# madmann91/bvh

Hardware: AMD Instinct MI355X
Metric: Mrays/s closest-hit (1M-tri scene) (higher is better)
Workload: dtype f32; 1 GPU; soup_1m: 1,000,000-triangle random soup (M3), worst-case incoherent; robust traversal, DefaultBuilder with thread pool (mini-trees) Quality::High built on the GPU (the reference's default configuration is thread pool + High); rays reordered for coherence inside the timed pass (library default for this tree size); tris=1000000, nodes=1866439, ray_batches=4, parallelism=single GPU, launched_by=single process

## Files before the change

bvh_amd/__init__.py:

```python
from .api import (BinnedSahBuilder, MiniTreeBuilder, SplitHeuristic, Bvh, Config, DefaultBuilder, Quality, RayFlags, SweepSahBuilder, ThreadPool, prepare_trace,
                  HITD, HITF, INVALID, NODED, NODEF, NODE2D, NODE2F, closest_points, hits_to_numpy, intersect, precompute_tris, sphere_bounds,
                  tri_bounds, gather, radius_count, radius_search, offsets_from_counts, knn, KNN_MAX_K, std_sort_ids, radix_sort_pairs, reinsertion_stats, last_optimize_profile, pinhole_rays, shade_eyelight)
from ._lib import BvhAmdError
```

bvh_amd/_lib.py:

```python
from __future__ import annotations

import ctypes as C
import os

HERE = os.path.dirname(os.path.abspath(__file__))
LIB_PATH = os.environ.get("BVH_AMD_LIB") or os.path.join(HERE, "lib", "libbvh_amd.so")

_lib = None


class BvhAmdError(RuntimeError):
    pass


class BuildConfig(C.Structure):
    _fields_ = [("quality", C.c_int), ("min_leaf_size", C.c_size_t), ("max_leaf_size", C.c_size_t),
                ("parallel_threshold", C.c_size_t)]


class Counters(C.Structure):
    _fields_ = [("node_pairs", C.c_ulonglong), ("prim_tests", C.c_ulonglong), ("leaves", C.c_ulonglong)]


class MiniTreeConfig(C.Structure):
# ... 106 lines not shown
    "bvh{S}_get_prim_id": (_Z, [_P, _Z]),
    "bvh{S}_get_prim_count": (_Z, [_P]),
    "bvh{S}_get_node_count": (_Z, [_P]),
    "bvh_node{S}_is_leaf": (C.c_bool, [_P]),
    "bvh_node{S}_get_prim_count": (_Z, [_P]),
    "bvh_node{S}_get_first_id": (_Z, [_P]),
    "bvh{S}_copy_nodes": (None, [_P, _P]),
    "bvh{S}_copy_prim_ids": (None, [_P, _P]),
    "bvh{S}_device_prim_ids": (_P, [_P]),
    "bvh_amd_tri_bounds{S}": (_I, [_P, _Z, _P, _P, _P]),
    "bvh_amd_precompute_tris{S}": (_I, [_P, _P, _Z, _P, _P]),
    "bvh_amd_sphere_bounds{S}": (_I, [_P, _Z, _P, _P, _P]),
    "bvh{S}_intersect_rays_tri": (_I, [_P, _P, _P, _Z, _U, _P, _P, _P]),
    "bvh{S}_intersect_rays_sphere": (_I, [_P, _P, _P, _Z, _U, _P, _P, _P]),
    "bvh{S}_prepare_trace": (_I, [_P, _Z, _P]),
    "bvh{S}_closest_points_tri": (_I, [_P, _P, _P, _Z, _U, _P, _P, _P]),
    "bvh{S}_closest_points_sphere": (_I, [_P, _P, _P, _Z, _U, _P, _P, _P]),
    "bvh{S}_radius_search_tri": (_I, [_P, _P, _P, _Z, _U, _P, _P, _P, _P, _P, _P]),
    "bvh{S}_radius_search_sphere": (_I, [_P, _P, _P, _Z, _U, _P, _P, _P, _P, _P, _P]),
    "bvh{S}_knn_tri": (_I, [_P, _P, _P, _Z, _U, _U, _P, _P, _P, _P, _P]),
    "bvh{S}_knn_sphere": (_I, [_P, _P, _P, _Z, _U, _U, _P, _P, _P, _P, _P]),
    "bvh{S}_intersect_ray": (None, [_P, _P, _P]),
    "bvh{S}_intersect_ray_any": (None, [_P, _P, _P]),
    "bvh{S}_intersect_ray_robust": (None, [_P, _P, _P]),
    "bvh{S}_intersect_ray_any_robust": (None, [_P, _P, _P]),
    "bvh{S}_intersect_ray_visit": (_I, [_P, _P, _Z, _U, _P]),
}


class OptimizeProfile(C.Structure):
# ... 6 lines not shown

class OptimizeConfig(C.Structure):
    _fields_ = [("batch_size_ratio", C.c_double), ("max_iter_count", C.c_size_t)]


def ray_visitor_types(suffix: str):
    scalar = C.c_float if suffix[1] == "f" else C.c_double
    leaf_t = C.CFUNCTYPE(C.c_bool, C.c_void_p, C.POINTER(scalar), C.c_size_t, C.c_size_t)
    inner_t = C.CFUNCTYPE(None, C.c_void_p, C.c_size_t)

    class Visitor(C.Structure):
        _fields_ = [("user_data", C.c_void_p), ("leaf_fn", leaf_t), ("inner_fn", inner_t)]
    return Visitor, leaf_t, inner_t


_ONLY_3D = ("bvh_amd_tri_bounds{S}", "bvh_amd_precompute_tris{S}", "bvh{S}_intersect_rays_tri", "bvh{S}_prepare_trace",
            "bvh{S}_build_minitree_device",
            "bvh{S}_closest_points_tri", "bvh{S}_closest_points_sphere",
            "bvh{S}_radius_search_tri", "bvh{S}_radius_search_sphere",
            "bvh{S}_knn_tri", "bvh{S}_knn_sphere",
            "bvh{S}_refit_tris", "bvh{S}_traversal_cost")


def exported_symbols():
    names = list(_SIGS)
    for s in ("3f", "3d", "2f", "2d"):
        names += [k.format(S=s) for k in _SIGS_T if s[0] == "3" or k not in _ONLY_3D]
        names += [f"bvh_node{s}_get_bbox"]
    return names


# ... 34 lines not shown
```

bvh_amd/api.py:

```python
from __future__ import annotations

import ctypes as C
import enum
from dataclasses import dataclass, field

import numpy as np

from . import _lib

INVALID = 0xFFFFFFFF
HITF = np.dtype([("prim", "<u4"), ("t", "<f4"), ("u", "<f4"), ("v", "<f4")])
HITD = np.dtype([("prim", "<u4"), ("pad", "<u4"), ("t", "<f8"), ("u", "<f8"), ("v", "<f8")])
NODEF = np.dtype([("bounds", "<f4", (6,)), ("index", "<u4")])
NODED = np.dtype([("bounds", "<f8", (6,)), ("index", "<u8")])
NODE2F = np.dtype([("bounds", "<f4", (4,)), ("index", "<u4")])
NODE2D = np.dtype([("bounds", "<f8", (4,)), ("index", "<u8")])
_NODE_DTYPES = {"3f": NODEF, "3d": NODED, "2f": NODE2F, "2d": NODE2D}


class Quality(enum.IntEnum):
    Low = 0
    Medium = 1
    High = 2

# ... 396 lines not shown

def gather(records, perm):
    torch = _torch()
    r = _dev(records)
    p = _dev(perm).to(torch.int32)
    out = torch.empty((p.shape[0],) + tuple(r.shape[1:]), dtype=r.dtype, device=r.device)
    stride = r.element_size() * int(np.prod(r.shape[1:]))
    _lib.check(_lib.load().bvh_amd_gather(r.data_ptr(), p.data_ptr(), p.shape[0], stride, out.data_ptr(), _stream()), "gather")
    return out


def prepare_trace(bvh: Bvh, n_rays_hint: int = 0):
    if bvh.dim != 3:
        return
    _lib.check(getattr(_lib.load(), f"bvh{bvh._s}_prepare_trace")(bvh._h, int(n_rays_hint), _stream()), "prepare_trace")


def intersect(bvh: Bvh, prims, rays, any_hit: bool = False, robust: bool = False, leaf: str = "tri",
              counters: bool = False, out=None, sort_rays=None, original_ids: bool = False):
    torch = _torch()
    lib = _lib.load()
    s = bvh._s
    dt = torch.float32 if s[1] == "f" else torch.float64
    r = _dev(rays, 2 * bvh.dim + 2)
    p = _dev(prims)
    if bvh.dim == 2:
        leaf = "sphere"
    if r.dtype != dt or p.dtype != dt:
        raise TypeError("prims/rays dtype must match the BVH scalar type")
    n = r.shape[0]
# ... 209 lines not shown
```

bvh_amd/csrc/capi.hip:

```cpp
#include "common.h"

#include <cstring>
#include <memory>

namespace bvh_amd {

template <typename T> int reinsertion_optimize_device(HostNode<T>* d_nodes, size_t node_count, hipStream_t stream, int dim);
template <typename T>
int reinsertion_optimize_config_device(HostNode<T>* d_nodes, size_t node_count, hipStream_t stream, int dim, double batch_size_ratio, size_t iterations);
void reinsertion_stats(unsigned out[2]);
void last_optimize_profile(bvh_amd_optimize_profile* out);
template <typename T>
int build_minitree_explicit(BvhImpl<T>& out, const T* d_bboxes, const T* d_centers, size_t n, const bvh_build_config& cfg, bool prune, T ratio,
                            bool optimize, uint32_t log2_grid, hipStream_t stream);
template <typename T>
int extract_device(BvhImpl<T>& out, const HostNode<T>* d_nodes, size_t node_count, const uint32_t* d_ids, size_t root_id, hipStream_t stream);
template <typename T> int refit_device(HostNode<T>* d_nodes, size_t node_count, hipStream_t stream);
template <typename T> int reachable_node_count(const HostNode<T>* d_nodes, size_t node_count, hipStream_t stream, size_t* out);
template <typename T> int relayout_on_device(BvhImpl<T>& b, const HostNode<T>* d_nodes, hipStream_t stream);

namespace {
thread_local std::string g_error;
}

// ... 289 lines not shown
        return fail(BVH_AMD_ERR_ARG, std::string(who) + ": " + std::to_string(n_src) + " primitives given, but prim_ids refers to primitive " +
                    std::to_string(b.max_prim_id) + " (the array is indexed by original primitive id)");
    const bool from_host = b.host_valid || !b.d_nodes || b.d_nodes_count != b.node_count;
    int rc = from_host ? b.wait_refit() : BVH_AMD_OK;
    if (rc) return rc;
    rc = make_nodes_resident<T>(b);
    if (rc) return rc;
    if (from_host || (b.pair_count && !b.d_pairs)) {
        const long long largest = b.max_prim_id;
        rc = relayout_on_device<T>(b, b.d_nodes, stream);
        if (rc) return rc;
        b.max_prim_id = largest;
    }
    rc = refit_prims_device<T>(b.d_nodes, b.d_pairs, b.node_count, src_kind, d_src, n_src, b.d_prim_ids, b.prim_count, stream);
    if (rc == BVH_AMD_OK && d_tris12_out) rc = launch_precompute_tris<T>(d_src, b.d_prim_ids, b.prim_count, d_tris12_out, stream);
    b.host_valid = false;
    b.nodes2_valid = false;
    const int rc2 = b.note_refit(stream);
    return rc ? rc : rc2;
}

template <typename T>
int traversal_cost_checked(const BvhImpl<T>* b, double* cost_out, void* stream) {
    if (!b || !cost_out) return fail(BVH_AMD_ERR_ARG, "traversal_cost: null bvh or output");
    int cur = -1;
    BVH_HIP_TRY(hipGetDevice(&cur), BVH_AMD_ERR_HIP);
    if (cur != b->device) return fail(BVH_AMD_ERR_ARG, "traversal_cost: BVH lives on another device than the current one");
    return traversal_cost<T>(*b, cost_out, static_cast<hipStream_t>(stream));
}

// ... 407 lines not shown
        return radius_search<T>(b, LEAF_TRIANGLE, prims, queries, n, flags, counts, offsets, list_prims, list_dist, cnt, s); } \
    int bvh##S##_radius_search_sphere(const bvh##S* b, const T* prims, const T* queries, size_t n, unsigned flags, uint32_t* counts, \
                                      const uint64_t* offsets, uint32_t* list_prims, T* list_dist, bvh_amd_counters* cnt, void* s) { \
        return radius_search<T>(b, LEAF_SPHERE, prims, queries, n, flags, counts, offsets, list_prims, list_dist, cnt, s); } \
    int bvh##S##_knn_tri(const bvh##S* b, const T* prims, const T* queries, size_t n, unsigned k, unsigned flags, uint32_t* out_prims, \
                         T* out_dist, uint32_t* counts, bvh_amd_counters* cnt, void* s) {                           \
        return knn<T>(b, LEAF_TRIANGLE, prims, queries, n, k, flags, out_prims, out_dist, counts, cnt, s); }        \
    int bvh##S##_knn_sphere(const bvh##S* b, const T* prims, const T* queries, size_t n, unsigned k, unsigned flags, uint32_t* out_prims, \
                            T* out_dist, uint32_t* counts, bvh_amd_counters* cnt, void* s) {                        \
        return knn<T>(b, LEAF_SPHERE, prims, queries, n, k, flags, out_prims, out_dist, counts, cnt, s); }          \
    int bvh##S##_prepare_trace(const bvh##S* b, size_t n_rays_hint, void* s) {                                      \
        if (!b) return fail(BVH_AMD_ERR_ARG, "prepare_trace: null bvh");                                            \
        int cur = -1;                                                                                               \
        BVH_HIP_TRY(hipGetDevice(&cur), BVH_AMD_ERR_HIP);                                                           \
        if (cur != impl<T>(b)->device) return fail(BVH_AMD_ERR_ARG, "prepare_trace: BVH lives on another device than the current one"); \
        return prepare_trace<T>(*impl<T>(b), n_rays_hint, static_cast<hipStream_t>(s)); }

BVH_AMD_IMPL(float, 3f)
BVH_AMD_IMPL(double, 3d)

#define BVH_AMD_IMPL_RAY(T, S, CB, VIS, D, IMPL)                                                                         \
    void bvh##S##_intersect_ray(const bvh##S* b, const bvh_ray##S* r, const CB* cb) { intersect_ray_legacy<T, D>(IMPL<T>(b), r, cb, 0u); } \
    void bvh##S##_intersect_ray_any(const bvh##S* b, const bvh_ray##S* r, const CB* cb) {                           \
        intersect_ray_legacy<T, D>(IMPL<T>(b), r, cb, BVH_AMD_RAY_ANY_HIT); }                                        \
    void bvh##S##_intersect_ray_robust(const bvh##S* b, const bvh_ray##S* r, const CB* cb) {                        \
        intersect_ray_legacy<T, D>(IMPL<T>(b), r, cb, BVH_AMD_RAY_ROBUST); }                                         \
    void bvh##S##_intersect_ray_any_robust(const bvh##S* b, const bvh_ray##S* r, const CB* cb) {                    \
        intersect_ray_legacy<T, D>(IMPL<T>(b), r, cb, BVH_AMD_RAY_ANY_HIT | BVH_AMD_RAY_ROBUST); }                   \
    int bvh##S##_intersect_ray_visit(const bvh##S* b, const bvh_ray##S* r, size_t start, unsigned flags, const VIS* v) { \
        if (!v || !v->leaf_fn) return fail(BVH_AMD_ERR_ARG, "intersect_ray_visit: null visitor");                   \
        return intersect_ray_visit<T, D>(IMPL<T>(b), r, start, flags, v->leaf_fn, v->inner_fn, v->user_data); }
// ... 127 lines not shown
```

bvh_amd/csrc/common.h:

```cpp
#pragma once

#include <hip/hip_runtime.h>

#include <cstddef>
#include <cstdint>
#include <cstring>
#include <string>
#include <atomic>
#include <mutex>
#include <vector>

#include "../../include/bvh_amd.h"

namespace bvh_amd {

constexpr unsigned kCountBits = 4;
constexpr uint32_t kCountMask = 15u;
constexpr int kWave = 64;

template <typename T> struct IndexOf;
template <> struct IndexOf<float>  { using Type = uint32_t; };
template <> struct IndexOf<double> { using Type = uint64_t; };

template <typename T>
// ... 69 lines not shown
    int sync_host() const;
    HostNode<T>* h_root = nullptr;
    hipEvent_t refit_done = nullptr;
    mutable std::atomic<bool> root_pending{false};
    mutable std::mutex root_mutex;
    int wait_refit() const;
    int note_refit(hipStream_t stream);
    long long max_prim_id = -1;
    int device = -1;
    PairNode<T>* d_pairs = nullptr;
    size_t pair_count = 0;
    uint32_t* d_prim_ids = nullptr;
    uint32_t root_index = 0;
    mutable std::atomic<int> max_depth{-1};
    mutable std::atomic<float> expected_visits{0.0f};
    mutable std::atomic<uint32_t> launch_plan[2] = {};
    struct PlanSearch {
        int index = 0;
        static constexpr int kCandidates = 5;
        int trying = -1;
        uint8_t count[kCandidates] = {};
        uint8_t dropped = 0;
        bool pending = false;
        bool recorded = false;
        hipEvent_t start = nullptr, stop = nullptr;
        size_t rays = 0;
        float ns_per_ray[kCandidates] = {};
        size_t rays_of[kCandidates] = {};
    };
    mutable PlanSearch plan_search[2];
// ... 132 lines not shown
```

bvh_amd/csrc/trace_body.inc:

```
#ifndef BVH_TRACE_COOP
#define BVH_TRACE_COOP false
#endif
    constexpr int kDepth = kLdsDepth;
    constexpr int kSpill = 64 - kDepth;
    __shared__ uint32_t lds_stack[kDepth * kBlock];
    uint32_t spill[kSpill];
    const int tid = threadIdx.x;
    const int lane = tid & (kWave - 1);
    const uint64_t lanes_below = (uint64_t{1} << lane) - 1;

    bool have = false, done = false, drained = false, nan_ray = false;
    uint32_t part = a.parts > 1 ? blockIdx.x % a.parts : 0, parts_left = a.parts;
    unsigned long long ray_id = 0;
    T org[3], dir[3], inv[3], aux[3];
    T tmin = 0, tmax = 0;
    uint32_t oct[3] = {0, 0, 0};
    uint32_t top = 0, sp = 0;
    uint32_t hit_prim = BVH_AMD_INVALID;
    T hit_t = 0, hit_u = 0, hit_v = 0;
    unsigned long long n_pairs = 0, n_tests = 0, n_leaves = 0;
#if defined(BVH_AMD_DEVELOPER) && defined(__HIPCC__)
    unsigned long long wt_begin = 0, wt_last_refill = 0, wt_rays = 0, wt_refill_ticks = 0, wt_refills = 0;
    if (a.wave_times) wt_begin = __builtin_amdgcn_s_memrealtime();
#endif

    auto deep_slot = [&](uint32_t i) { return a.deep + (size_t{blockIdx.x} * kBlock + tid) * a.deep_cap + i; };
    auto push = [&](uint32_t v) {
        if (sp < kDepth) lds_stack[sp * kBlock + tid] = v;
        else if (!Deep) spill[min(sp - kDepth, static_cast<uint32_t>(kSpill - 1))] = v;
        else if (sp < kDepth + kSpill) spill[sp - kDepth] = v;
        else *deep_slot(min(sp - (kDepth + kSpill), a.deep_cap - 1)) = v;
        ++sp;
    };
    auto pop = [&]() -> uint32_t {
        --sp;
        uint32_t v = lds_word(&lds_stack[min(sp, static_cast<uint32_t>(kDepth - 1)) * kBlock + tid]);
        if (sp >= kDepth) {
            if (!Deep) v = spill[min(sp - kDepth, static_cast<uint32_t>(kSpill - 1))];
            else if (sp < kDepth + kSpill) v = spill[sp - kDepth];
            else v = *deep_slot(min(sp - (kDepth + kSpill), a.deep_cap - 1));
        }
        return v;
    };

    for (;;) {
        const uint64_t idle = __ballot(!have);
        const int n_idle = __popcll(idle);
        if (!drained && (n_idle >= a.refill_threshold || n_idle == kWave)) {
#if defined(BVH_AMD_DEVELOPER) && defined(__HIPCC__)
            unsigned long long wt_t0 = 0;
            if (a.wave_times) wt_t0 = __builtin_amdgcn_s_memrealtime();
// ... 51 lines not shown
                wt_refill_ticks += wt_last_refill - wt_t0; ++wt_refills;
            }
#endif
        }
        if (__ballot(have) == 0) {
            if (drained) break;
            continue;
        }

        for (;;) {
            const bool inner = have && !done && (top & kCountMask) == 0;
            const uint64_t inner_mask = __ballot(inner);
            if (!inner_mask) break;
            const int parked = __popcll(__ballot(have && !done && (top & kCountMask) != 0));
            if (parked >= a.leaf_threshold) break;
            T lb[6], rb[6];
            uint32_t li = 0, ri = 0;
            if constexpr (BVH_TRACE_COOP) coop_load_pair(a.pairs, a.pair_bytes, inner ? (top >> (kCountBits + 1)) : 0xFFFFFFFFu, lane, lb, rb, li, ri);
            if (inner) {
                if constexpr (!BVH_TRACE_COOP) load_pair(a.pairs + (top >> (kCountBits + 1)), lb, rb, li, ri);
                if (Stats) ++n_pairs;
                T l0 = tmin, l1 = tmax, r0 = tmin, r1 = tmax;
#pragma unroll
                for (int k = 0; k < D; ++k) {
                    const T ln = oct[k] ? lb[2 * k + 1] : lb[2 * k], lf = oct[k] ? lb[2 * k] : lb[2 * k + 1];
                    const T rn = oct[k] ? rb[2 * k + 1] : rb[2 * k], rf = oct[k] ? rb[2 * k] : rb[2 * k + 1];
                    T la, lz, ra, rz;
                    if (Robust) {
                        la = (ln - org[k]) * inv[k]; lz = (lf - org[k]) * aux[k];
                        ra = (rn - org[k]) * inv[k]; rz = (rf - org[k]) * aux[k];
                    } else {
                        la = Num<T>::fma_(ln, inv[k], aux[k]); lz = Num<T>::fma_(lf, inv[k], aux[k]);
                        ra = Num<T>::fma_(rn, inv[k], aux[k]); rz = Num<T>::fma_(rf, inv[k], aux[k]);
                    }
                    l0 = Num<T>::max_num(la, l0); l1 = Num<T>::min_num(lz, l1);
                    r0 = Num<T>::max_num(ra, r0); r1 = Num<T>::min_num(rz, r1);
                }
                const bool hl = !nan_ray && l0 <= l1, hr = !nan_ray && r0 <= r1;
                if (hl) {
                    uint32_t near_i = li;
                    if (hr) {
                        uint32_t far_i = ri;
                        if (!Any && l0 > r0) { near_i = ri; far_i = li; }
                        push(far_i);
                    }
                    top = near_i;
                } else if (hr) {
                    top = ri;
                } else if (sp == 0) {
                    done = true;
                } else {
                    top = pop();
                }
            }
        }

        if (have && !done && (top & kCountMask) != 0) {
            const uint32_t first = top >> kCountBits, count = top & kCountMask;
            if (Stats) ++n_leaves;
// ... 77 lines not shown
```

bvh_amd/csrc/trace_device.h:

```cpp
#pragma once

#if defined(__HIPCC__)
#define BVH_AMD_KEEP_APART(v) asm volatile("" : "+v"(v))
#else
#define BVH_AMD_KEEP_APART(v) asm volatile("" : "+r"(v))
#endif

namespace bvh_amd {

namespace {

constexpr int kBlock = 256;
constexpr int kLdsDepth = 20;
constexpr int kRefillThreshold = 36;
constexpr int kRefillThresholdSmall = 20;
constexpr int kLeafThreshold = 12;
constexpr int kCoopRefillAny = 20, kCoopLeafAny = 20;
constexpr int kCoopRefillHeavy = 12, kCoopLeafHeavy = 12;


template <typename T> struct Num;
template <> struct Num<float> {
    static constexpr float kMax = 3.402823466e+38f, kEps = 1.1920928955078125e-07f;
    __device__ static bool finite(float x) { return (__float_as_uint(x) & 0x7F800000u) != 0x7F800000u; }
    __device__ static float bump2(float x) { return __uint_as_float(__float_as_uint(x) + 2u); }
    __device__ static bool sign(float x) { return (__float_as_uint(x) >> 31) != 0; }
    __device__ static float fma_(float a, float b, float c) { return __builtin_fmaf(a, b, c); }
    __device__ static float sqrt_(float x) { return __builtin_sqrtf(x); }
// ... 20 lines not shown
template <typename T> __device__ inline T pick_min(T a, T b) { return a < b ? a : b; }
template <typename T> __device__ inline T pick_max(T a, T b) { return a > b ? a : b; }

template <typename T> __device__ inline T dot3(T a0, T a1, T a2, T b0, T b1, T b2) {
    return ((T(0) + a0 * b0) + a1 * b1) + a2 * b2;
}
__device__ inline uint32_t lds_word(const uint32_t* shared) {
#if defined(__HIP_DEVICE_COMPILE__)
    typedef __attribute__((address_space(3))) const volatile uint32_t LdsWord;
    return *(LdsWord*)shared;
#else
    return *shared;
#endif
}

template <typename T> __device__ inline T dot2(T a0, T a1, T b0, T b1) { return (T(0) + a0 * b0) + a1 * b1; }

constexpr uint32_t kTicketStride = 16;

template <typename T>
struct TraceArgs {
    const PairNode<T>* pairs;
    const T* prims;
    const T* rays;
    typename HitOf<T>::Type* hits;
    unsigned long long n;
    unsigned long long* work;
    unsigned long long part_size;
    uint32_t parts;
    bvh_amd_counters* counters;
    const uint32_t* order;
    uint32_t* deep;
    uint32_t deep_cap;
    uint32_t root_index;
    int refill_threshold;
    int leaf_threshold;
    uint32_t coop;
    uint32_t prim_stride;
    uint32_t stream_hints;
    uint32_t stagger;
    uint32_t one_shot;
    unsigned long long* wave_times;
    uint32_t pair_bytes = 0;
};

__device__ inline void load_pair(const PairNode<float>* p, float (&lb)[6], float (&rb)[6], uint32_t& li, uint32_t& ri) {
    const float4* q = reinterpret_cast<const float4*>(p);
    float4 a = q[0], b = q[1], c = q[2];
    uint2 d = reinterpret_cast<const uint2*>(p)[6];
    lb[0] = a.x; lb[1] = a.y; lb[2] = a.z; lb[3] = a.w; lb[4] = b.x; lb[5] = b.y;
    rb[0] = b.z; rb[1] = b.w; rb[2] = c.x; rb[3] = c.y; rb[4] = c.z; rb[5] = c.w;
    li = d.x; ri = d.y;
}
__device__ inline void load_pair(const PairNode<double>* p, double (&lb)[6], double (&rb)[6], uint32_t& li, uint32_t& ri) {
    const double2* q = reinterpret_cast<const double2*>(p);
#pragma unroll
    for (int i = 0; i < 3; ++i) { double2 v = q[i]; lb[2 * i] = v.x; lb[2 * i + 1] = v.y; }
#pragma unroll
// ... 198 lines not shown
```

bvh_amd/csrc/traverse.hip:

```cpp

#include "common.h"
#include "trace_device.h"
#include "ray_key.h"

#include <algorithm>
#include <chrono>
#include <cstdlib>
#include <cstring>
#include <memory>
#include <mutex>
#include <thread>
#include <type_traits>
#include <vector>

namespace bvh_amd {

namespace {

thread_local const char* g_last_kernel = "";
thread_local bool g_last_reordered = false;
thread_local int g_last_plan[4] = {0, 0, 0, 0};

struct KernelTimer {
    static constexpr size_t kRing = 256;
// ... 107 lines not shown
    path <<= (depth - level);
    const uint32_t oct = (Num<float>::sign(r[3]) ? 1u : 0u) | (Num<float>::sign(r[4]) ? 2u : 0u) | (Num<float>::sign(r[5]) ? 4u : 0u);
    keys[i] = (path << 3) | oct;
}

template <typename H>
__global__ void __launch_bounds__(256) original_ids_kernel(H* hits, size_t n, const uint32_t* prim_ids, uint32_t prim_count) {
    const size_t i = blockIdx.x * size_t{256} + threadIdx.x;
    if (i >= n) return;
    const uint32_t p = hits[i].prim;
    if (p < prim_count) hits[i].prim = prim_ids[p];
}

thread_local int t_refill = -1, t_leaf = -1, t_coop = -1, t_parts = -1;
struct Experiments { int grid_blocks = -1, stream_hints = -1, tri_stride = -1, key_curve = -1, key_bits = -1, step_events = -1, wave_times = -1, one_shot = -1,
                     key_class_bits = -1, key_class_scale = -1, stagger = -1; };
constexpr int kKeyClassBits = 0, kKeyClassScalePercent = 500;
constexpr uint32_t kStaggerHeavy = 100000, kStaggerLight = 50000, kStaggerDouble = 20000;
thread_local bool g_last_classes = false;
thread_local float g_search_ns[5] = {0, 0, 0, 0, 0};
thread_local int g_search_count[5] = {0, 0, 0, 0, 0};
thread_local unsigned g_search_dropped = 0;
thread_local Experiments t_exp;
#if defined(BVH_AMD_DEVELOPER)
constexpr size_t kWaveTimeWords = 6, kWaveTimeWaves = 8 * 256 * (kBlock / kWave) * 2;
thread_local unsigned long long* t_wave_times = nullptr;
thread_local size_t t_wave_times_waves = 0;
#endif
thread_local std::pair<hipEvent_t, hipEvent_t>* t_calibration = nullptr;

int coop_fetch_forced() {
// ... 282 lines not shown

}

void last_launch_plan(int out[4]) { for (int k = 0; k < 4; ++k) out[k] = g_last_plan[k]; }
void set_tuning(int refill, int leaf, int coop, int parts) { t_refill = refill; t_leaf = leaf; t_coop = coop; t_parts = parts; }
int set_experiment(const char* name, int value) {
    const std::string k = name ? name : "";
    if (k == "grid_blocks") t_exp.grid_blocks = value;
    else if (k == "stream_hints") t_exp.stream_hints = value;
    else if (k == "tri_stride") t_exp.tri_stride = value;
    else if (k == "key_curve") t_exp.key_curve = value;
    else if (k == "key_bits") t_exp.key_bits = value;
    else if (k == "step_events") t_exp.step_events = value;
    else if (k == "one_shot") t_exp.one_shot = value;
    else if (k == "stagger") t_exp.stagger = value;
    else if (k == "key_class_bits") t_exp.key_class_bits = value;
    else if (k == "key_class_scale") t_exp.key_class_scale = value;
    else if (k == "wave_times") {
#if defined(BVH_AMD_DEVELOPER)
        t_exp.wave_times = value;
#else
        return fail(BVH_AMD_ERR_ARG, "bvh_amd_experiment: 'wave_times' exists in the developer library only (python -m bvh_amd.build --developer)");
#endif
    }
    else if (k == "reset") t_exp = Experiments{};
    else return fail(BVH_AMD_ERR_ARG, "bvh_amd_experiment: unknown knob '" + k + "'");
    return BVH_AMD_OK;
}
int wave_times(unsigned long long* out, size_t capacity_waves, size_t* n_waves) {
#if defined(BVH_AMD_DEVELOPER)
// ... 115 lines not shown
    auto release = [&](int rc) {
        (void)hipEventRecord(slot_event, stream);
        { std::lock_guard<std::mutex> lock(b.work_mutex); b.work_busy[slot] = false; }
        if (deep_mem) scratch_free(deep_mem, deep_tag);
        if (sort_mem) scratch_free(sort_mem, sort_tag);
        return rc;
    };
    if (d_counters) {
        const hipError_t e = hipMemsetAsync(d_counters, 0, sizeof(bvh_amd_counters), stream);
        if (e != hipSuccess) return release(fail(BVH_AMD_ERR_HIP, std::string("intersect_rays: hipMemsetAsync: ") + hipGetErrorString(e)));
    }
    {
        int rc = tree_depth<T>(b, stream);
        if (rc) return release(rc);
        const int max_depth = b.max_depth.load();
        if (max_depth > 64) {
            int cus = 0;
            if (hipDeviceGetAttribute(&cus, hipDeviceAttributeMultiprocessorCount, b.device) != hipSuccess) return release(fail(BVH_AMD_ERR_HIP, "intersect_rays: hipDeviceGetAttribute"));
            const size_t lanes = size_t{8} * cus * kBlock;
            const size_t cap = static_cast<size_t>(max_depth - 64 + 1);
            if (lanes * cap > (size_t{1} << 32))
                return release(fail(BVH_AMD_ERR_UNSUPPORTED, "intersect_rays: the tree is too deep for the traversal stack (" + std::to_string(max_depth) + " levels)"));
            const hipError_t e = scratch_alloc(&deep_mem, lanes * cap * sizeof(uint32_t), &deep_tag);
            if (e != hipSuccess) { deep_mem = nullptr; return release(fail(BVH_AMD_ERR_HIP, std::string("intersect_rays: stack spill buffer: ") + hipGetErrorString(e))); }
            args.deep = static_cast<uint32_t*>(deep_mem); args.deep_cap = static_cast<uint32_t>(cap);
            args.one_shot = 0;
        }
    }
    static const int refill_env = BVH_DEV_INT("BVH_AMD_REFILL", 0);
    static const int leaf_env = BVH_DEV_INT("BVH_AMD_LEAF", 0);
    const bool beyond_l2 = b.pair_count * sizeof(PairNode<T>) > (size_t{32} << 20);
    const bool heavy = beyond_l2 && b.expected_visits.load() >= kReorderMinVisits;
    const bool any_hit = (flags & BVH_AMD_RAY_ANY_HIT) != 0;
    const int forced = coop_fetch_forced();
    const bool coop_capable = true;
// ... 377 lines not shown
```

bvh_amd/csrc/upload.hip:

```cpp
#include "common.h"

#include <mutex>

namespace bvh_amd {

namespace {

template <typename T>
__global__ void __launch_bounds__(256) relayout_pairs(const HostNode<T>* nodes, size_t pair_count, PairNode<T>* out) {
    size_t p = blockIdx.x * size_t{256} + threadIdx.x;
    if (p >= pair_count) return;
    const HostNode<T>& l = nodes[2 * p + 1];
    const HostNode<T>& r = nodes[2 * p + 2];
    PairNode<T> rec;
#pragma unroll
    for (int k = 0; k < 6; ++k) { rec.lb[k] = l.bounds[k]; rec.rb[k] = r.bounds[k]; }
    rec.li = static_cast<uint32_t>(l.index);
    rec.ri = static_cast<uint32_t>(r.index);
#pragma unroll
    for (size_t k = 0; k < sizeof(rec.pad) / 4; ++k) rec.pad[k] = 0;
    out[p] = rec;
}

template <typename T>
// ... 29 lines not shown
        auto share = [&](const T* b, uint32_t index) -> unsigned long long {
            if ((index & kCountMask) != 0) return 0;
            const double x = double(b[1]) - double(b[0]), y = double(b[3]) - double(b[2]), z = double(b[5]) - double(b[4]);
            const double r = (x * y + y * z + z * x) * inv_root_area;
            return r > 0 ? static_cast<unsigned long long>(fmin(r, 1.0) * 65536.0) : 0;
        };
        mine = share(q.lb, q.li) + share(q.rb, q.ri);
    }
    __shared__ unsigned long long part[4];
    for (int off = 32; off > 0; off >>= 1) mine += __shfl_down(mine, off);
    if ((threadIdx.x & 63) == 0) part[threadIdx.x >> 6] = mine;
    __syncthreads();
    if (threadIdx.x == 0) atomicAdd(sum, part[0] + part[1] + part[2] + part[3]);
}

}

template <typename T>
int tree_depth(const BvhImpl<T>& b, hipStream_t stream) {
    if (b.max_depth.load() >= 0) return BVH_AMD_OK;
    static std::mutex once;
    std::lock_guard<std::mutex> lock(once);
    if (b.max_depth.load() >= 0) return BVH_AMD_OK;
    if (b.pair_count == 0) { b.max_depth = 0; return BVH_AMD_OK; }
    if (const int rc = b.wait_refit()) return rc;
    const uint32_t n = static_cast<uint32_t>(b.pair_count);
    StreamScope scratch_on(stream);
    ScratchTag buf_tag;
    uint32_t* buf = nullptr;
    BVH_HIP_TRY(scratch_alloc(reinterpret_cast<void**>(&buf), (size_t{4} * n + 4) * sizeof(uint32_t), &buf_tag), BVH_AMD_ERR_HIP);
    uint32_t *anc = buf, *dist = buf + n, *anc2 = buf + 2 * size_t{n}, *dist2 = buf + 3 * size_t{n};
    uint32_t* d_max = buf + 4 * size_t{n};
    unsigned long long* d_visits = reinterpret_cast<unsigned long long*>(d_max + 2);
    hipError_t e = hipMemsetAsync(d_max, 0, 16, stream);
    const unsigned grid = (n + 255) / 256;
    {
        const double x = double(b.root_bounds[1]) - double(b.root_bounds[0]), y = double(b.root_bounds[3]) - double(b.root_bounds[2]),
                     z = b.dim == 3 ? double(b.root_bounds[5]) - double(b.root_bounds[4]) : 0.0;
        const double area = x * y + y * z + z * x;
        hipLaunchKernelGGL(k_expected_visits<T>, dim3(grid), dim3(256), 0, stream, b.d_pairs, n, area > 0 ? 1.0 / area : 0.0, d_visits);
    }
    hipLaunchKernelGGL(k_depth_identity, dim3(grid), dim3(256), 0, stream, n, anc, dist);
    hipLaunchKernelGGL(k_depth_init<T>, dim3(grid), dim3(256), 0, stream, b.d_pairs, n, b.root_index >> (kCountBits + 1), anc, dist);
    int rounds = 1;
    while ((uint64_t{1} << rounds) < uint64_t{n} + 1) ++rounds;
    uint32_t words[4] = {0, 0, 0, 0};
    int done = 0;
    for (const int upto : {std::min(rounds, 7), rounds}) {
        if (done >= upto) break;
        if (done) e = hipMemsetAsync(d_max, 0, 8, stream);
        for (int r = done; r < upto; ++r) {
            hipLaunchKernelGGL(k_depth_jump, dim3(grid), dim3(256), 0, stream, anc, dist, n, anc2, dist2, r == upto - 1 ? d_max : nullptr,
                               b.root_index >> (kCountBits + 1));
            std::swap(anc, anc2); std::swap(dist, dist2);
        }
        done = upto;
        if (e == hipSuccess) e = hipGetLastError();
        if (e == hipSuccess) e = hipMemcpyAsync(words, d_max, 16, hipMemcpyDeviceToHost, stream);
        if (e == hipSuccess) e = hipStreamSynchronize(stream);
        if (e != hipSuccess || words[1] == 0) break;
    }
    scratch_free(buf, buf_tag);
    if (e != hipSuccess) return fail(BVH_AMD_ERR_HIP, std::string("tree_depth: ") + hipGetErrorString(e));
    const uint32_t deepest = words[0];
    b.expected_visits = static_cast<float>(static_cast<double>((static_cast<unsigned long long>(words[3]) << 32) | words[2]) / 65536.0);
    b.max_depth = static_cast<int>(deepest) + 1;
    return BVH_AMD_OK;
}
template int tree_depth<float>(const BvhImpl<float>&, hipStream_t);
template int tree_depth<double>(const BvhImpl<double>&, hipStream_t);

template <typename T>
BvhImpl<T>::~BvhImpl() {
    if (device >= 0) {
        int cur = -1;
        (void)hipGetDevice(&cur);
        if (cur != device) (void)hipSetDevice(device);
        if (d_pairs) { scratch_forget(d_pairs); (void)hipFree(d_pairs); }
        if (d_prim_ids) { scratch_forget(d_prim_ids); (void)hipFree(d_prim_ids); }
        if (d_work) (void)hipFree(d_work);
// ... 72 lines not shown
    std::vector<uint32_t> ids(prim_count);
    hipError_t e = hipMemcpy(nodes.data(), d_nodes, node_count * sizeof(HostNode<T>), hipMemcpyDeviceToHost);
    if (e == hipSuccess) e = hipMemcpy(ids.data(), d_prim_ids, prim_count * sizeof(uint32_t), hipMemcpyDeviceToHost);
    if (cur != device) (void)hipSetDevice(cur);
    if (e != hipSuccess) return fail(BVH_AMD_ERR_HIP, std::string("sync_host: ") + hipGetErrorString(e));
    prim_ids.assign(ids.begin(), ids.end());
    nodes2_valid.store(false);
    host_valid.store(true, std::memory_order_release);
    return BVH_AMD_OK;
}

template <typename T>
int relayout_on_device(BvhImpl<T>& b, const HostNode<T>* d_nodes, hipStream_t stream) {
    b.pair_count = (b.node_count - 1) / 2;
    b.max_depth = -1;
    b.max_prim_id = -1;
    { std::lock_guard<std::mutex> lock(b.plan_mutex); for (int k = 0; k < 2; ++k) { b.launch_plan[k] = 0; b.plan_search[k].index = 0; b.plan_search[k].pending = false; b.plan_search[k].trying = -1; b.plan_search[k].dropped = 0; for (auto& c : b.plan_search[k].count) c = 0; for (auto& t : b.plan_search[k].ns_per_ray) t = 0.0f; for (auto& r : b.plan_search[k].rays_of) r = 0; } }
    if (b.d_pairs) { scratch_forget(b.d_pairs); (void)hipFree(b.d_pairs); b.d_pairs = nullptr; }
    if (b.pair_count) {
        StreamScope scratch_on(stream);
        ScratchTag tag;
        BVH_HIP_TRY(scratch_alloc(reinterpret_cast<void**>(&b.d_pairs), b.pair_count * sizeof(PairNode<T>), &tag), BVH_AMD_ERR_HIP);
        unsigned grid = static_cast<unsigned>((b.pair_count + 255) / 256);
        hipLaunchKernelGGL(relayout_pairs<T>, dim3(grid), dim3(256), 0, stream, d_nodes, b.pair_count, b.d_pairs);
        BVH_HIP_TRY(hipGetLastError(), BVH_AMD_ERR_HIP);
    }
    return BVH_AMD_OK;
}

template <typename T>
// ... 66 lines not shown
```

include/bvh_amd.h:

```cpp
#ifndef BVH_AMD_H
#define BVH_AMD_H

#include <stddef.h>
#include <stdint.h>
#include <stdio.h>
#include <stdbool.h>

#ifdef __cplusplus
extern "C" {
#endif

#define BVH_AMD_API __attribute__((visibility("default")))

#define BVH_ROOT_INDEX 0
#define BVH_INVALID_PRIM_ID SIZE_MAX

struct bvh3f;
struct bvh3d;
struct bvh_node3f;
struct bvh_node3d;
struct bvh2f;
struct bvh2d;
struct bvh_node2f;
struct bvh_node2d;
// ... 274 lines not shown
    uint32_t* d_counts, const uint64_t* d_offsets, uint32_t* d_list_prims, double* d_list_dist, struct bvh_amd_counters* d_counters, void* stream);
BVH_AMD_API int bvh_amd_offsets_from_counts(const uint32_t* d_counts, size_t n, uint64_t* d_offsets, void* stream);

#define BVH_AMD_KNN_MAX_K 64
BVH_AMD_API int bvh3f_knn_tri(const struct bvh3f*, const float* d_tris12, const float* d_queries4, size_t n, unsigned k, unsigned flags,
    uint32_t* d_out_prims, float* d_out_dist, uint32_t* d_counts, struct bvh_amd_counters* d_counters, void* stream);
BVH_AMD_API int bvh3d_knn_tri(const struct bvh3d*, const double* d_tris12, const double* d_queries4, size_t n, unsigned k, unsigned flags,
    uint32_t* d_out_prims, double* d_out_dist, uint32_t* d_counts, struct bvh_amd_counters* d_counters, void* stream);
BVH_AMD_API int bvh3f_knn_sphere(const struct bvh3f*, const float* d_sph4, const float* d_queries4, size_t n, unsigned k, unsigned flags,
    uint32_t* d_out_prims, float* d_out_dist, uint32_t* d_counts, struct bvh_amd_counters* d_counters, void* stream);
BVH_AMD_API int bvh3d_knn_sphere(const struct bvh3d*, const double* d_sph4, const double* d_queries4, size_t n, unsigned k, unsigned flags,
    uint32_t* d_out_prims, double* d_out_dist, uint32_t* d_counts, struct bvh_amd_counters* d_counters, void* stream);

BVH_AMD_API int bvh3f_prepare_trace(const struct bvh3f*, size_t n_rays_hint, void* stream);
BVH_AMD_API int bvh3d_prepare_trace(const struct bvh3d*, size_t n_rays_hint, void* stream);

BVH_AMD_API int bvh_amd_std_sort_ids3f(const float* d_keys, size_t n, uint32_t* d_ids_out, void* stream);
BVH_AMD_API int bvh_amd_std_sort_ids3d(const double* d_keys, size_t n, uint32_t* d_ids_out, void* stream);
BVH_AMD_API int bvh_amd_radix_sort_pairs_u32(uint32_t* d_keys, uint32_t* d_vals, size_t n, int bits, void* stream);

BVH_AMD_API const char* bvh_amd_last_kernel_name(void);
BVH_AMD_API int bvh_amd_last_launch_reordered(void);
BVH_AMD_API void bvh_amd_kernel_timing(int on);
BVH_AMD_API int bvh_amd_kernel_times(float* ms_out, size_t capacity, size_t* count_out);
BVH_AMD_API int bvh_amd_reorder_times(float* ms_out, size_t capacity, size_t* count_out);
BVH_AMD_API void bvh_amd_tuning(int refill_threshold, int leaf_threshold, int coop_fetch, int ticket_ranges);
BVH_AMD_API int bvh_amd_experiment(const char* name, int value);
BVH_AMD_API int bvh_amd_wave_times(unsigned long long* out, size_t capacity_waves, size_t* n_waves);
BVH_AMD_API void bvh_amd_last_launch_plan(int out[4]);
BVH_AMD_API void bvh_amd_last_plan_search(float ns_per_ray[5], int measurements[5], unsigned* dropped_mask);
// ... 136 lines not shown
```

Before: 2443 Mrays/s.

## Store entry distance on LDS stack and skip stale popped nodes in nested trees

The traversal stack now keeps each pushed far child together with its entry distance as a uint2 in LDS. On pop, if that distance already exceeds the current tmax, the child pair fetch and box tests are skipped. This is allowed only when a new device check confirms every child box sits inside its parent box. The LDS depth is halved to 10 with a 44-entry register spill, which doubles LDS bytes per slot and moves the deep-stack threshold. The change adds a nestedness kernel to the tree-depth pass and a tree_nested query to the API.

```diff
diff --git a/bvh_amd/__init__.py b/bvh_amd/__init__.py
--- a/bvh_amd/__init__.py
+++ b/bvh_amd/__init__.py
@@ -1,4 +1,4 @@
-from .api import (BinnedSahBuilder, MiniTreeBuilder, SplitHeuristic, Bvh, Config, DefaultBuilder, Quality, RayFlags, SweepSahBuilder, ThreadPool, prepare_trace,
+from .api import (BinnedSahBuilder, MiniTreeBuilder, SplitHeuristic, Bvh, Config, DefaultBuilder, Quality, RayFlags, SweepSahBuilder, ThreadPool, prepare_trace, tree_nested,
                   HITD, HITF, INVALID, NODED, NODEF, NODE2D, NODE2F, closest_points, hits_to_numpy, intersect, precompute_tris, sphere_bounds,
                   tri_bounds, gather, radius_count, radius_search, offsets_from_counts, knn, KNN_MAX_K, std_sort_ids, radix_sort_pairs, reinsertion_stats, last_optimize_profile, pinhole_rays, shade_eyelight)
 from ._lib import BvhAmdError
diff --git a/bvh_amd/_lib.py b/bvh_amd/_lib.py
--- a/bvh_amd/_lib.py
+++ b/bvh_amd/_lib.py
@@ -144,6 +144,7 @@
     "bvh{S}_intersect_rays_tri": (_I, [_P, _P, _P, _Z, _U, _P, _P, _P]),
     "bvh{S}_intersect_rays_sphere": (_I, [_P, _P, _P, _Z, _U, _P, _P, _P]),
     "bvh{S}_prepare_trace": (_I, [_P, _Z, _P]),
+    "bvh{S}_tree_nested": (_I, [_P, _P, _P]),
     "bvh{S}_closest_points_tri": (_I, [_P, _P, _P, _Z, _U, _P, _P, _P]),
     "bvh{S}_closest_points_sphere": (_I, [_P, _P, _P, _Z, _U, _P, _P, _P]),
     "bvh{S}_radius_search_tri": (_I, [_P, _P, _P, _Z, _U, _P, _P, _P, _P, _P, _P]),
@@ -180,7 +181,7 @@
     return Visitor, leaf_t, inner_t
 
 
-_ONLY_3D = ("bvh_amd_tri_bounds{S}", "bvh_amd_precompute_tris{S}", "bvh{S}_intersect_rays_tri", "bvh{S}_prepare_trace",
+_ONLY_3D = ("bvh_amd_tri_bounds{S}", "bvh_amd_precompute_tris{S}", "bvh{S}_intersect_rays_tri", "bvh{S}_prepare_trace", "bvh{S}_tree_nested",
             "bvh{S}_build_minitree_device",
             "bvh{S}_closest_points_tri", "bvh{S}_closest_points_sphere",
             "bvh{S}_radius_search_tri", "bvh{S}_radius_search_sphere",
diff --git a/bvh_amd/api.py b/bvh_amd/api.py
--- a/bvh_amd/api.py
+++ b/bvh_amd/api.py
@@ -434,6 +434,13 @@
     if bvh.dim != 3:
         return
     _lib.check(getattr(_lib.load(), f"bvh{bvh._s}_prepare_trace")(bvh._h, int(n_rays_hint), _stream()), "prepare_trace")
+
+
+def tree_nested(bvh: Bvh) -> bool:
+    import ctypes
+    flag = ctypes.c_int(0)
+    _lib.check(getattr(_lib.load(), f"bvh{bvh._s}_tree_nested")(bvh._h, ctypes.byref(flag), _stream()), "tree_nested")
+    return bool(flag.value)
 
 
 def intersect(bvh: Bvh, prims, rays, any_hit: bool = False, robust: bool = False, leaf: str = "tri",
diff --git a/bvh_amd/csrc/capi.hip b/bvh_amd/csrc/capi.hip
--- a/bvh_amd/csrc/capi.hip
+++ b/bvh_amd/csrc/capi.hip
@@ -327,6 +327,7 @@
     }
     rc = refit_prims_device<T>(b.d_nodes, b.d_pairs, b.node_count, src_kind, d_src, n_src, b.d_prim_ids, b.prim_count, stream);
     if (rc == BVH_AMD_OK && d_tris12_out) rc = launch_precompute_tris<T>(d_src, b.d_prim_ids, b.prim_count, d_tris12_out, stream);
+    b.nested = 0;
     b.host_valid = false;
     b.nodes2_valid = false;
     const int rc2 = b.note_refit(stream);
@@ -764,7 +765,15 @@
         int cur = -1;                                                                                               \
         BVH_HIP_TRY(hipGetDevice(&cur), BVH_AMD_ERR_HIP);                                                           \
         if (cur != impl<T>(b)->device) return fail(BVH_AMD_ERR_ARG, "prepare_trace: BVH lives on another device than the current one"); \
-        return prepare_trace<T>(*impl<T>(b), n_rays_hint, static_cast<hipStream_t>(s)); }
+        return prepare_trace<T>(*impl<T>(b), n_rays_hint, static_cast<hipStream_t>(s)); }                               \
+    int bvh##S##_tree_nested(const bvh##S* b, int* nested, void* s) {                                               \
+        if (!b || !nested) return fail(BVH_AMD_ERR_ARG, "tree_nested: null bvh or output");                         \
+        int cur = -1;                                                                                               \
+        BVH_HIP_TRY(hipGetDevice(&cur), BVH_AMD_ERR_HIP);                                                           \
+        if (cur != impl<T>(b)->device) return fail(BVH_AMD_ERR_ARG, "tree_nested: BVH lives on another device than the current one"); \
+        if (impl<T>(b)->node_count && impl<T>(b)->d_pairs) { if (const int rc = tree_depth<T>(*impl<T>(b), static_cast<hipStream_t>(s))) return rc; } \
+        *nested = impl<T>(b)->nested.load();                                                                        \
+        return BVH_AMD_OK; }
 
 BVH_AMD_IMPL(float, 3f)
 BVH_AMD_IMPL(double, 3d)
diff --git a/bvh_amd/csrc/common.h b/bvh_amd/csrc/common.h
--- a/bvh_amd/csrc/common.h
+++ b/bvh_amd/csrc/common.h
@@ -107,6 +107,7 @@
     uint32_t root_index = 0;
     mutable std::atomic<int> max_depth{-1};
     mutable std::atomic<float> expected_visits{0.0f};
+    mutable std::atomic<int> nested{0};
     mutable std::atomic<uint32_t> launch_plan[2] = {};
     struct PlanSearch {
         int index = 0;
diff --git a/bvh_amd/csrc/trace_body.inc b/bvh_amd/csrc/trace_body.inc
--- a/bvh_amd/csrc/trace_body.inc
+++ b/bvh_amd/csrc/trace_body.inc
@@ -1,9 +1,11 @@
 #ifndef BVH_TRACE_COOP
 #define BVH_TRACE_COOP false
 #endif
-    constexpr int kDepth = kLdsDepth;
-    constexpr int kSpill = 64 - kDepth;
-    __shared__ uint32_t lds_stack[kDepth * kBlock];
+    constexpr bool kKeyed = !Any;
+    constexpr int kDepth = kKeyed ? kLdsDepth : 2 * kLdsDepth;
+    constexpr int kSpill = kSpillDepth;
+    __shared__ uint2 lds_stack[kLdsDepth * kBlock];
+    uint32_t* const lds_words = reinterpret_cast<uint32_t*>(lds_stack);
     uint32_t spill[kSpill];
     const int tid = threadIdx.x;
     const int lane = tid & (kWave - 1);
@@ -25,8 +27,11 @@
 #endif
 
     auto deep_slot = [&](uint32_t i) { return a.deep + (size_t{blockIdx.x} * kBlock + tid) * a.deep_cap + i; };
-    auto push = [&](uint32_t v) {
-        if (sp < kDepth) lds_stack[sp * kBlock + tid] = v;
+    auto push = [&](uint32_t v, T entry) {
+        if (sp < kDepth) {
+            if constexpr (kKeyed) lds_stack[sp * kBlock + tid] = make_uint2(v, stack_distance(entry));
+            else lds_words[sp * kBlock + tid] = v;
+        }
         else if (!Deep) spill[min(sp - kDepth, static_cast<uint32_t>(kSpill - 1))] = v;
         else if (sp < kDepth + kSpill) spill[sp - kDepth] = v;
         else *deep_slot(min(sp - (kDepth + kSpill), a.deep_cap - 1)) = v;
@@ -34,7 +39,14 @@
     };
     auto pop = [&]() -> uint32_t {
         --sp;
-        uint32_t v = lds_word(&lds_stack[min(sp, static_cast<uint32_t>(kDepth - 1)) * kBlock + tid]);
+        uint32_t v;
+        if constexpr (kKeyed) {
+            const uint2 w = lds_pair(&lds_stack[min(sp, static_cast<uint32_t>(kDepth - 1)) * kBlock + tid]);
+            v = w.x;
+            if (a.nested && (v & kCountMask) == 0 && static_cast<T>(__uint_as_float(w.y)) > tmax) v = kStaleTop;
+        } else {
+            v = lds_word(&lds_words[min(sp, static_cast<uint32_t>(kDepth - 1)) * kBlock + tid]);
+        }
         if (sp >= kDepth) {
             if (!Deep) v = spill[min(sp - kDepth, static_cast<uint32_t>(kSpill - 1))];
             else if (sp < kDepth + kSpill) v = spill[sp - kDepth];
@@ -116,12 +128,13 @@
             if (!inner_mask) break;
             const int parked = __popcll(__ballot(have && !done && (top & kCountMask) != 0));
             if (parked >= a.leaf_threshold) break;
-            T lb[6], rb[6];
+            const bool stale = kKeyed && top == kStaleTop;
+            T lb[6] = {}, rb[6] = {};
             uint32_t li = 0, ri = 0;
-            if constexpr (BVH_TRACE_COOP) coop_load_pair(a.pairs, a.pair_bytes, inner ? (top >> (kCountBits + 1)) : 0xFFFFFFFFu, lane, lb, rb, li, ri);
+            if constexpr (BVH_TRACE_COOP) coop_load_pair(a.pairs, a.pair_bytes, inner && !stale ? (top >> (kCountBits + 1)) : 0xFFFFFFFFu, lane, lb, rb, li, ri);
             if (inner) {
-                if constexpr (!BVH_TRACE_COOP) load_pair(a.pairs + (top >> (kCountBits + 1)), lb, rb, li, ri);
-                if (Stats) ++n_pairs;
+                if constexpr (!BVH_TRACE_COOP) { if (!stale) load_pair(a.pairs + (top >> (kCountBits + 1)), lb, rb, li, ri); }
+                if (Stats && !(stale && a.count_fetches)) ++n_pairs;
                 T l0 = tmin, l1 = tmax, r0 = tmin, r1 = tmax;
 #pragma unroll
                 for (int k = 0; k < D; ++k) {
@@ -138,13 +151,15 @@
                     l0 = Num<T>::max_num(la, l0); l1 = Num<T>::min_num(lz, l1);
                     r0 = Num<T>::max_num(ra, r0); r1 = Num<T>::min_num(rz, r1);
                 }
-                const bool hl = !nan_ray && l0 <= l1, hr = !nan_ray && r0 <= r1;
+                const bool live = !nan_ray && !stale;
+                const bool hl = live && l0 <= l1, hr = live && r0 <= r1;
                 if (hl) {
                     uint32_t near_i = li;
                     if (hr) {
                         uint32_t far_i = ri;
-                        if (!Any && l0 > r0) { near_i = ri; far_i = li; }
-                        push(far_i);
+                        T far_e = r0;
+                        if (!Any && l0 > r0) { near_i = ri; far_i = li; far_e = l0; }
+                        push(far_i, far_e);
                     }
                     top = near_i;
                 } else if (hr) {
diff --git a/bvh_amd/csrc/trace_device.h b/bvh_amd/csrc/trace_device.h
--- a/bvh_amd/csrc/trace_device.h
+++ b/bvh_amd/csrc/trace_device.h
@@ -11,7 +11,14 @@
 namespace {
 
 constexpr int kBlock = 256;
-constexpr int kLdsDepth = 20;
+constexpr int kLdsDepth = 10;
+#if defined(__HIPCC__)
+constexpr int kSpillDepth = 44;
+#else
+constexpr int kSpillDepth = 64 - kLdsDepth;
+#endif
+constexpr int kSmallStack = kLdsDepth + kSpillDepth;
+constexpr uint32_t kStaleTop = 0xFFFFFFE0u;
 constexpr int kRefillThreshold = 36;
 constexpr int kRefillThresholdSmall = 20;
 constexpr int kLeafThreshold = 12;
@@ -62,6 +69,26 @@
 #endif
 }
 
+__device__ inline uint2 lds_pair(const uint2* shared) {
+#if defined(__HIP_DEVICE_COMPILE__)
+    typedef __attribute__((address_space(3))) const volatile unsigned long long LdsPair;
+    const unsigned long long v = *(LdsPair*)shared;
+    return make_uint2(static_cast<uint32_t>(v), static_cast<uint32_t>(v >> 32));
+#else
+    return *shared;
+#endif
+}
+__device__ inline uint32_t stack_distance(float e) { return __float_as_uint(e); }
+__device__ inline uint32_t stack_distance(double e) {
+#if defined(__HIP_DEVICE_COMPILE__)
+    return __float_as_uint(__double2float_rd(e));
+#else
+    float f = static_cast<float>(e);
+    if (static_cast<double>(f) > e) f = __builtin_nextafterf(f, -__builtin_inff());
+    return __float_as_uint(f);
+#endif
+}
+
 template <typename T> __device__ inline T dot2(T a0, T a1, T b0, T b1) { return (T(0) + a0 * b0) + a1 * b1; }
 
 constexpr uint32_t kTicketStride = 16;
@@ -90,6 +117,8 @@
     uint32_t one_shot;
     unsigned long long* wave_times;
     uint32_t pair_bytes = 0;
+    uint32_t nested = 0;
+    uint32_t count_fetches = 0;
 };
 
 __device__ inline void load_pair(const PairNode<float>* p, float (&lb)[6], float (&rb)[6], uint32_t& li, uint32_t& ri) {
diff --git a/bvh_amd/csrc/traverse.hip b/bvh_amd/csrc/traverse.hip
--- a/bvh_amd/csrc/traverse.hip
+++ b/bvh_amd/csrc/traverse.hip
@@ -145,7 +145,7 @@
 
 thread_local int t_refill = -1, t_leaf = -1, t_coop = -1, t_parts = -1;
 struct Experiments { int grid_blocks = -1, stream_hints = -1, tri_stride = -1, key_curve = -1, key_bits = -1, step_events = -1, wave_times = -1, one_shot = -1,
-                     key_class_bits = -1, key_class_scale = -1, stagger = -1; };
+                     key_class_bits = -1, key_class_scale = -1, stagger = -1, stale_skip = -1, count_fetches = -1; };
 constexpr int kKeyClassBits = 0, kKeyClassScalePercent = 500;
 constexpr uint32_t kStaggerHeavy = 100000, kStaggerLight = 50000, kStaggerDouble = 20000;
 thread_local bool g_last_classes = false;
@@ -458,6 +458,8 @@
     else if (k == "step_events") t_exp.step_events = value;
     else if (k == "one_shot") t_exp.one_shot = value;
     else if (k == "stagger") t_exp.stagger = value;
+    else if (k == "stale_skip") t_exp.stale_skip = value;
+    else if (k == "count_fetches") t_exp.count_fetches = value;
     else if (k == "key_class_bits") t_exp.key_class_bits = value;
     else if (k == "key_class_scale") t_exp.key_class_scale = value;
     else if (k == "wave_times") {
@@ -603,11 +605,13 @@
         int rc = tree_depth<T>(b, stream);
         if (rc) return release(rc);
         const int max_depth = b.max_depth.load();
-        if (max_depth > 64) {
+        args.nested = b.nested.load() == 1 && !(flags & BVH_AMD_RAY_ANY_HIT) && t_exp.stale_skip != 0 ? 1u : 0u;
+        args.count_fetches = t_exp.count_fetches > 0 ? 1u : 0u;
+        if (max_depth > kSmallStack) {
             int cus = 0;
             if (hipDeviceGetAttribute(&cus, hipDeviceAttributeMultiprocessorCount, b.device) != hipSuccess) return release(fail(BVH_AMD_ERR_HIP, "intersect_rays: hipDeviceGetAttribute"));
             const size_t lanes = size_t{8} * cus * kBlock;
-            const size_t cap = static_cast<size_t>(max_depth - 64 + 1);
+            const size_t cap = static_cast<size_t>(max_depth - kSmallStack + 1);
             if (lanes * cap > (size_t{1} << 32))
                 return release(fail(BVH_AMD_ERR_UNSUPPORTED, "intersect_rays: the tree is too deep for the traversal stack (" + std::to_string(max_depth) + " levels)"));
             const hipError_t e = scratch_alloc(&deep_mem, lanes * cap * sizeof(uint32_t), &deep_tag);
diff --git a/bvh_amd/csrc/upload.hip b/bvh_amd/csrc/upload.hip
--- a/bvh_amd/csrc/upload.hip
+++ b/bvh_amd/csrc/upload.hip
@@ -67,6 +67,25 @@
     if (threadIdx.x == 0) atomicAdd(sum, part[0] + part[1] + part[2] + part[3]);
 }
 
+template <typename T>
+__global__ void __launch_bounds__(256) k_not_nested(const PairNode<T>* pairs, uint32_t n_pairs, uint32_t* violated) {
+    const uint32_t p = blockIdx.x * 256 + threadIdx.x;
+    if (p >= n_pairs) return;
+    const PairNode<T>& q = pairs[p];
+    auto inside = [&](const T* b, uint32_t index) {
+        if ((index & kCountMask) != 0) return true;
+        const uint32_t c = index >> (kCountBits + 1);
+        if (c >= n_pairs) return false;
+        const PairNode<T>& k = pairs[c];
+        bool ok = true;
+#pragma unroll
+        for (int x = 0; x < 3; ++x)
+            ok = ok && k.lb[2 * x] >= b[2 * x] && k.lb[2 * x + 1] <= b[2 * x + 1] && k.rb[2 * x] >= b[2 * x] && k.rb[2 * x + 1] <= b[2 * x + 1];
+        return ok;
+    };
+    if (!inside(q.lb, q.li) || !inside(q.rb, q.ri)) *violated = 1u;
+}
+
 }
 
 template <typename T>
@@ -75,17 +94,17 @@
     static std::mutex once;
     std::lock_guard<std::mutex> lock(once);
     if (b.max_depth.load() >= 0) return BVH_AMD_OK;
-    if (b.pair_count == 0) { b.max_depth = 0; return BVH_AMD_OK; }
+    if (b.pair_count == 0) { b.nested = 0; b.max_depth = 0; return BVH_AMD_OK; }
     if (const int rc = b.wait_refit()) return rc;
     const uint32_t n = static_cast<uint32_t>(b.pair_count);
     StreamScope scratch_on(stream);
     ScratchTag buf_tag;
     uint32_t* buf = nullptr;
-    BVH_HIP_TRY(scratch_alloc(reinterpret_cast<void**>(&buf), (size_t{4} * n + 4) * sizeof(uint32_t), &buf_tag), BVH_AMD_ERR_HIP);
+    BVH_HIP_TRY(scratch_alloc(reinterpret_cast<void**>(&buf), (size_t{4} * n + 8) * sizeof(uint32_t), &buf_tag), BVH_AMD_ERR_HIP);
     uint32_t *anc = buf, *dist = buf + n, *anc2 = buf + 2 * size_t{n}, *dist2 = buf + 3 * size_t{n};
     uint32_t* d_max = buf + 4 * size_t{n};
     unsigned long long* d_visits = reinterpret_cast<unsigned long long*>(d_max + 2);
-    hipError_t e = hipMemsetAsync(d_max, 0, 16, stream);
+    hipError_t e = hipMemsetAsync(d_max, 0, 32, stream);
     const unsigned grid = (n + 255) / 256;
     {
         const double x = double(b.root_bounds[1]) - double(b.root_bounds[0]), y = double(b.root_bounds[3]) - double(b.root_bounds[2]),
@@ -93,11 +112,12 @@
         const double area = x * y + y * z + z * x;
         hipLaunchKernelGGL(k_expected_visits<T>, dim3(grid), dim3(256), 0, stream, b.d_pairs, n, area > 0 ? 1.0 / area : 0.0, d_visits);
     }
+    hipLaunchKernelGGL(k_not_nested<T>, dim3(grid), dim3(256), 0, stream, b.d_pairs, n, d_max + 4);
     hipLaunchKernelGGL(k_depth_identity, dim3(grid), dim3(256), 0, stream, n, anc, dist);
     hipLaunchKernelGGL(k_depth_init<T>, dim3(grid), dim3(256), 0, stream, b.d_pairs, n, b.root_index >> (kCountBits + 1), anc, dist);
     int rounds = 1;
     while ((uint64_t{1} << rounds) < uint64_t{n} + 1) ++rounds;
-    uint32_t words[4] = {0, 0, 0, 0};
+    uint32_t words[8] = {0, 0, 0, 0, 1, 0, 0, 0};
     int done = 0;
     for (const int upto : {std::min(rounds, 7), rounds}) {
         if (done >= upto) break;
@@ -109,7 +129,7 @@
         }
         done = upto;
         if (e == hipSuccess) e = hipGetLastError();
-        if (e == hipSuccess) e = hipMemcpyAsync(words, d_max, 16, hipMemcpyDeviceToHost, stream);
+        if (e == hipSuccess) e = hipMemcpyAsync(words, d_max, 32, hipMemcpyDeviceToHost, stream);
         if (e == hipSuccess) e = hipStreamSynchronize(stream);
         if (e != hipSuccess || words[1] == 0) break;
     }
@@ -117,6 +137,7 @@
     if (e != hipSuccess) return fail(BVH_AMD_ERR_HIP, std::string("tree_depth: ") + hipGetErrorString(e));
     const uint32_t deepest = words[0];
     b.expected_visits = static_cast<float>(static_cast<double>((static_cast<unsigned long long>(words[3]) << 32) | words[2]) / 65536.0);
+    b.nested = words[4] == 0 ? 1 : 0;
     b.max_depth = static_cast<int>(deepest) + 1;
     return BVH_AMD_OK;
 }
@@ -219,6 +240,7 @@
 int relayout_on_device(BvhImpl<T>& b, const HostNode<T>* d_nodes, hipStream_t stream) {
     b.pair_count = (b.node_count - 1) / 2;
     b.max_depth = -1;
+    b.nested = 0;
     b.max_prim_id = -1;
     { std::lock_guard<std::mutex> lock(b.plan_mutex); for (int k = 0; k < 2; ++k) { b.launch_plan[k] = 0; b.plan_search[k].index = 0; b.plan_search[k].pending = false; b.plan_search[k].trying = -1; b.plan_search[k].dropped = 0; for (auto& c : b.plan_search[k].count) c = 0; for (auto& t : b.plan_search[k].ns_per_ray) t = 0.0f; for (auto& r : b.plan_search[k].rays_of) r = 0; } }
     if (b.d_pairs) { scratch_forget(b.d_pairs); (void)hipFree(b.d_pairs); b.d_pairs = nullptr; }
diff --git a/include/bvh_amd.h b/include/bvh_amd.h
--- a/include/bvh_amd.h
+++ b/include/bvh_amd.h
@@ -312,6 +312,8 @@
 
 BVH_AMD_API int bvh3f_prepare_trace(const struct bvh3f*, size_t n_rays_hint, void* stream);
 BVH_AMD_API int bvh3d_prepare_trace(const struct bvh3d*, size_t n_rays_hint, void* stream);
+BVH_AMD_API int bvh3f_tree_nested(const struct bvh3f*, int* nested, void* stream);
+BVH_AMD_API int bvh3d_tree_nested(const struct bvh3d*, int* nested, void* stream);
 
 BVH_AMD_API int bvh_amd_std_sort_ids3f(const float* d_keys, size_t n, uint32_t* d_ids_out, void* stream);
 BVH_AMD_API int bvh_amd_std_sort_ids3d(const double* d_keys, size_t n, uint32_t* d_ids_out, void* stream);
```

Measured after the change: 2412 Mrays/s. -1.3%, worse.
